# isgasho/h2o-kubernetes

Measured on AMD Instinct MI355X. Metric: GBM train rows/sec on HIGGS-shape 11M×28 at 1/2/4/8 MI355X; AUC parity, higher is better.
Workload: dtype fp32 gradients/hessians; histograms in fixed-point int32 (stochastic rounding) summed exactly in int64; fp64 split gains; exact int64 leaf sums; uint8 bins; 1 GPU; model=GBM bernoulli, global_batch=11000000, rows_per_gpu=11000000, cols=28, max_depth=5, nbins=255, parallelism=dp1

## Files before the change

### h2omx/csrc/tree_kernels.hip

```cpp
#include "common.h"
#include "p2p_device.h"
#include <math.h>

#include <algorithm>
#include <cstdlib>

namespace {

struct SplitParams {
  int mode;
  int leaf_mode;
  int F;
  int is_last_level;
  double min_rows;
  double min_child_weight;
  double lambda_;
  double alpha;
  double gamma;
  double min_split_improvement;
  double learn_rate;
  double max_abs_leaf;
  uint32_t seed;
  int tree_index;
  int depth;
// ... 635 lines not shown
    }
    const unsigned long long bal = __ballot(do_split);
    if (i < n)
      lf_write_node(i, s, do_split, __popcll(bal & ((1ull << lane) - 1ull)), base, next_base, p, nbt, lv, writer,
                    ps_s + i);
    if (lane == 0) {
      int ks = __popcll(bal);
      if (writer) lf_write_ctl(lv.ctl_next, ks, next_base, lv.max_next_nodes);
      if (2 * ks > lv.max_next_nodes) ks = lv.max_next_nodes / 2;
      *res_s = ks;
    }
  }
  __syncthreads();
  return *res_s;
}

struct LevelFin {
  LevelOut lv;
  int* ticket;
};

template <int MODE>
__device__ void level_fin_records(const FeatBest* __restrict__ fbest, const int* __restrict__ ctl, const SplitParams& p,
                                  int nbt, const LevelOut& lv) {
  const int n = ctl[CTL_N];
  const int lane = threadIdx.x & 63, wid = threadIdx.x >> 6, nw = blockDim.x >> 6;
  for (int node = wid; node < n; node += nw) node_best_wave<MODE>(fbest, p.F, node, lane, lv.nsplit);
  __syncthreads();
  level_finalize_body(ctl, p, nbt, lv);
}

constexpr int CMP_STAGE_BYTES = 2048;
constexpr int HB_PF = 1;

template <int NBT, int ROWS, int PKM, bool ROUTE, bool CMP, int COP = 1, bool NID16 = false>
__global__ __launch_bounds__(1024) void hist_build_kernel(
    const uint8_t* __restrict__ codes, int64_t npad, const float* __restrict__ g, const float* __restrict__ s2,
    const int* __restrict__ nid, const NodeLink* __restrict__ link, const int* __restrict__ ctl,
    const int* __restrict__ nvb, const double* __restrict__ qscale, uint32_t salt, int F, int fg, int n_groups,
    int wgpg, int slot_lo, int slot_cnt, const short* __restrict__ slot16, unsigned long long* __restrict__ pk_buf,
    unsigned long long* __restrict__ partials, const PartInfo* __restrict__ part_prev,
    const int* __restrict__ ctl_prev, int* __restrict__ nid_out, int writer, GradFuse gf, LevelPro lp,
    const uint8_t* __restrict__ joint, const int* __restrict__ plane_src) {
  salt = (uint32_t)qscale[9];
  extern __shared__ __attribute__((aligned(16))) unsigned long long lds64[];
  __shared__ int width_s[256], rep_s[256];
  __shared__ float rcp_s[256];
  __shared__ NodeSplit pro_ns[ROUTE ? PRO_MAX_NODES : 1];
  __shared__ PartInfo pro_ps[ROUTE ? PRO_MAX_NODES : 1];
  __shared__ int pro_res;
  bool pro = false;
  if constexpr (ROUTE) pro = lp.fbest != nullptr;
  int n_slots;
  if (pro) n_slots = level_prologue(lp, ctl_prev, NBT, blockIdx.x == 0 && writer != 0, pro_ns, pro_ps, &pro_res);
  else n_slots = ctl[CTL_SLOTS];
  const int b = blockIdx.x;
  const int xcd = b & 7, i = b >> 3;
  const int group = i % n_groups;
  const int chunk = xcd + 8 * (i / n_groups);
  const bool route_w = ROUTE && writer && group == 0 && ctl_prev[CTL_N] > 0;
  const bool build = slot_lo < n_slots;
  if (!build && !route_w) return;
  const int f0 = group * fg;
  const int nf = min(fg, F - f0);
  static_assert(COP == 1 || ((PKM == 1 || PKM == 3 || PKM == 6) && !ROUTE && !CMP), "copies: level-0 kernel only");
  const int hist_elems = slot_cnt * fg * NBT;
  const int lane = threadIdx.x & 63;
  auto plane_codes = [&](int fi) -> const uint8_t* {
    const int sp = plane_src ? plane_src[f0 + fi] : f0 + fi;
    return sp >= 0 ? codes + (int64_t)sp * npad : joint + (int64_t)(~sp) * npad;
  };

  for (int j = threadIdx.x; j < hist_elems * COP; j += blockDim.x) lds64[j] = 0ull;
  if (threadIdx.x < fg) {
    const int fi = threadIdx.x;
    const int w = (fi < nf) ? nvb[f0 + fi] + 1 : NBT;
    width_s[fi] = w;
    int r = NBT / w;
    r = r < 1 ? 1 : (r > 64 ? 64 : r);
    if (COP > 1) r = 1;
    rep_s[fi] = r;
    rcp_s[fi] = 1.0f / (float)r;
  }
  __shared__ float tval_s[PKM == 5 ? GF_LDS_NODES : 1];
  if constexpr (PKM == 5) {
    if (gf.apply && gf.cap <= GF_LDS_NODES)
      for (int j = threadIdx.x; j < gf.cap; j += blockDim.x) tval_s[j] = gf.tree[j].value;
  }
  const float sg = (float)qscale[0], ss = (float)qscale[1];
  const int64_t rb = (int64_t)qscale[7];
  const int64_t n_rows = (int64_t)qscale[8];
  __syncthreads();

  const int64_t units = npad / ROWS;
  const int64_t u0 = units * chunk / wgpg, u1 = units * (chunk + 1) / wgpg;
  const int64_t ustart = CMP ? u0 + (threadIdx.x & ~63) : u0 + threadIdx.x;
  for (int64_t uu = ustart; uu < u1; uu += blockDim.x) {
    const bool inb = !CMP || uu + lane < u1;
    const int64_t u = CMP ? (inb ? uu + lane : u1 - 1) : uu;
    const int64_t r0 = u * ROWS;
    int s[ROWS];
    bool any = false;
    if constexpr (ROUTE) {
      int nn[ROWS], nx[ROWS];
      if (nid == nullptr) {
#pragma unroll
        for (int k = 0; k < ROWS; ++k) nn[k] = (r0 + k < n_rows) ? 0 : INT32_MIN;
      } else if constexpr (NID16) {
        const short* n16 = reinterpret_cast<const short*>(nid);
#pragma unroll
        for (int q = 0; q < ROWS / 8; ++q) {
          const uint4 v = *reinterpret_cast<const uint4*>(n16 + r0 + 8 * q);
          const uint32_t w4[4] = {v.x, v.y, v.z, v.w};
#pragma unroll
          for (int k = 0; k < 8; ++k) nn[8 * q + k] = (int)(short)(w4[k >> 1] >> (16 * (k & 1)));
        }
      } else {
#pragma unroll
        for (int q = 0; q < ROWS / 4; ++q) {
          const int4 n4 = *reinterpret_cast<const int4*>(nid + r0 + 4 * q);
          nn[4 * q] = n4.x; nn[4 * q + 1] = n4.y; nn[4 * q + 2] = n4.z; nn[4 * q + 3] = n4.w;
        }
      }
#pragma unroll
      for (int k = 0; k < ROWS; ++k) { nx[k] = nn[k]; s[k] = -1; }
      const int n_prev = pro ? min(ctl_prev[CTL_N], PRO_MAX_NODES) : ctl_prev[CTL_N];
// ... 67 lines not shown
          any |= (sl >= 0);
        }
      }
    } else if (nid == nullptr) {
#pragma unroll
      for (int k = 0; k < ROWS; ++k) {
        int sl = (r0 + k < n_rows) ? 0 - slot_lo : -1;
        if (sl >= slot_cnt) sl = -1;
        s[k] = sl;
        any |= (sl >= 0);
      }
    } else {
#pragma unroll
      for (int q = 0; q < ROWS / 4; ++q) {
        const int4 n4 = *reinterpret_cast<const int4*>(nid + r0 + 4 * q);
        const int nn[4] = {n4.x, n4.y, n4.z, n4.w};
#pragma unroll
        for (int k = 0; k < 4; ++k) {
          int sl = -1;
          if (nn[k] >= 0) {
            sl = link[nn[k]].slot - slot_lo;
            if (sl >= slot_cnt) sl = -1;
          }
          s[4 * q + k] = sl;
          any |= (sl >= 0);
        }
      }
    }
    if constexpr (CMP) {
      if (__ballot(any && inb) == 0ull) continue;
    } else {
      if (!any) continue;
    }
    uint32_t pf[HB_PF][ROWS / 4];
    auto load_codes = [&](int fi, uint32_t* cw) {
      const uint8_t* cp = plane_codes(fi) + r0;
      if constexpr (ROWS == 16) {
        const uint4 c4 = *reinterpret_cast<const uint4*>(cp);
        cw[0] = c4.x; cw[1] = c4.y; cw[2] = c4.z; cw[3] = c4.w;
      } else {
        const uint2 c2 = *reinterpret_cast<const uint2*>(cp);
        cw[0] = c2.x; cw[1] = c2.y;
      }
    };
    if constexpr (!CMP) {
#pragma unroll
      for (int q = 0; q < HB_PF; ++q)
        if (q < nf) load_codes(q, pf[q]);
    }
    unsigned long long pk[ROWS];
    if constexpr (PKM == 2) {
#pragma unroll
      for (int q = 0; q < ROWS / 2; ++q) {
        const ulonglong2 p2 = *reinterpret_cast<const ulonglong2*>(pk_buf + r0 + 2 * q);
        pk[2 * q] = p2.x;
        pk[2 * q + 1] = p2.y;
      }
    } else if constexpr (PKM == 4 || PKM == 6) {
      const uint32_t* pk32 = reinterpret_cast<const uint32_t*>(pk_buf);
#pragma unroll
      for (int q = 0; q < ROWS / 4; ++q) {
        const uint4 p4 = *reinterpret_cast<const uint4*>(pk32 + r0 + 4 * q);
        const uint32_t pw[4] = {p4.x, p4.y, p4.z, p4.w};
#pragma unroll
        for (int k = 0; k < 4; ++k)
          pk[4 * q + k] = ((unsigned long long)(uint32_t)(int)(short)(pw[k] >> 16) << 32) |
                          (unsigned long long)(pw[k] & 0xFFFFu);
      }
    } else if constexpr (PKM == 5) {
#pragma unroll
      for (int q = 0; q < ROWS / 4; ++q) {
        const float4 f4 = *reinterpret_cast<const float4*>(gf.F + r0 + 4 * q);
        const float4 y4 = *reinterpret_cast<const float4*>(gf.y + r0 + 4 * q);
        int4 n4 = make_int4(-1, -1, -1, -1);
        if (gf.apply) n4 = *reinterpret_cast<const int4*>(gf.nid + r0 + 4 * q);
        float fv[4] = {f4.x, f4.y, f4.z, f4.w};
        const float yv[4] = {y4.x, y4.y, y4.z, y4.w};
        const int nv[4] = {n4.x, n4.y, n4.z, n4.w};
        float gv[4], hv[4];
        uint32_t pw[4];
#pragma unroll
        for (int k = 0; k < 4; ++k) {
          const int64_t r = r0 + 4 * q + k;
          gv[k] = 0.f; hv[k] = 0.f; pw[k] = 0u;
          pk[4 * q + k] = 0ull;
          if (r >= n_rows) continue;
          if (gf.apply) fv[k] += (gf.cap <= GF_LDS_NODES) ? tval_s[~nv[k]] : gf.tree[~nv[k]].value;
          dist_grad(gf.gp.dist, fv[k], yv[k], gf.gp, gv[k], hv[k]);
          const uint32_t hsh = row_hash(rb + r, salt);
          const float d1 = (hsh & 0xFFFF) * (1.0f / 65536.0f), d2 = (hsh >> 16) * (1.0f / 65536.0f);
          const int gq = (int)floorf(fmaf(gv[k], sg, d1));
          const uint32_t sq = (uint32_t)floorf(fmaf(gf.s_is_h ? hv[k] : 1.0f, ss, d2));
          pk[4 * q + k] = ((unsigned long long)(uint32_t)gq << 32) | (unsigned long long)sq;
          pw[k] = ((uint32_t)gq << 16) | (sq & 0xFFFFu);
        }
        if (group == 0) {
          if (gf.apply) *reinterpret_cast<float4*>(gf.F + r0 + 4 * q) = make_float4(fv[0], fv[1], fv[2], fv[3]);
          *reinterpret_cast<float4*>(gf.g + r0 + 4 * q) = make_float4(gv[0], gv[1], gv[2], gv[3]);
          *reinterpret_cast<float4*>(gf.h + r0 + 4 * q) = make_float4(hv[0], hv[1], hv[2], hv[3]);
          if (gf.pk64) {
            *reinterpret_cast<ulonglong2*>(pk_buf + r0 + 4 * q) = make_ulonglong2(pk[4 * q], pk[4 * q + 1]);
            *reinterpret_cast<ulonglong2*>(pk_buf + r0 + 4 * q + 2) = make_ulonglong2(pk[4 * q + 2], pk[4 * q + 3]);
          } else {
            *reinterpret_cast<uint4*>(reinterpret_cast<uint32_t*>(pk_buf) + r0 + 4 * q) =
                make_uint4(pw[0], pw[1], pw[2], pw[3]);
          }
        }
      }
    } else {
#pragma unroll
    for (int q = 0; q < ROWS / 4; ++q) {
      const float4 g4 = *reinterpret_cast<const float4*>(g + r0 + 4 * q);
      float4 s4 = make_float4(1.f, 1.f, 1.f, 1.f);
      if (s2) s4 = *reinterpret_cast<const float4*>(s2 + r0 + 4 * q);
      const float gv[4] = {g4.x, g4.y, g4.z, g4.w};
      const float sv[4] = {s4.x, s4.y, s4.z, s4.w};
#pragma unroll
      for (int k = 0; k < 4; ++k) {
        const uint32_t hsh = row_hash(rb + r0 + 4 * q + k, salt);
        const float d1 = (hsh & 0xFFFF) * (1.0f / 65536.0f), d2 = (hsh >> 16) * (1.0f / 65536.0f);
        const int gq = (int)floorf(fmaf(gv[k], sg, d1));
        const uint32_t sq = (uint32_t)floorf(fmaf(sv[k], ss, d2));
        pk[4 * q + k] = ((unsigned long long)(uint32_t)gq << 32) | (unsigned long long)sq;
      }
    }
    if (PKM == 1 && group == 0) {
#pragma unroll
      for (int q = 0; q < ROWS / 2; ++q)
        *reinterpret_cast<ulonglong2*>(pk_buf + r0 + 2 * q) = make_ulonglong2(pk[2 * q], pk[2 * q + 1]);
    }
    if (PKM == 3 && group == 0) {
      uint32_t* pk32 = reinterpret_cast<uint32_t*>(pk_buf);
#pragma unroll
      for (int q = 0; q < ROWS / 4; ++q) {
        uint32_t pw[4];
#pragma unroll
        for (int k = 0; k < 4; ++k) {
          const unsigned long long v = pk[4 * q + k];
          pw[k] = ((uint32_t)(v >> 32) << 16) | ((uint32_t)v & 0xFFFFu);
        }
        *reinterpret_cast<uint4*>(pk32 + r0 + 4 * q) = make_uint4(pw[0], pw[1], pw[2], pw[3]);
      }
    }
    }
    if constexpr (CMP) {
      static_assert(ROWS == 16 && (PKM == 2 || PKM == 4), "compaction: 16-row units reading stored rows");
      uint32_t m = 0;
#pragma unroll
      for (int r = 0; r < ROWS; ++r)
        if (inb && s[r] >= 0 && pk[r] != 0ull) m |= 1u << r;
      const uint32_t cnt = __popc(m);
      const unsigned long long lt = (1ull << lane) - 1ull;
      int excl = 0, total = 0;
#pragma unroll
      for (int bit = 0; bit < 5; ++bit) {
        const unsigned long long bm = __ballot((cnt >> bit) & 1u);
        excl += __popcll(bm & lt) << bit;
// ... 1644 lines not shown
  if (level_out == nullptr) return false;
  lv = *reinterpret_cast<const LevelOut*>(level_out);
  return lv.ctl_next != nullptr && lv.nvb != nullptr && lv.part != nullptr && lv.tree != nullptr &&
         lv.nsplit != nullptr;
}

static bool make_pro(LevelPro& lp, const void* fbest, const void* params, const void* level_out, int max_nodes) {
  if (fbest == nullptr || params == nullptr || max_nodes < 1 || max_nodes > PRO_MAX_NODES) return false;
  lp.fbest = reinterpret_cast<const FeatBest*>(fbest);
  lp.p = *reinterpret_cast<const SplitParams*>(params);
  return copy_level_out(lp.lv, level_out);
}

static int hist_build_launch(const uint8_t* codes, int64_t npad, const float* g, const float* s2, const int* nid,
                             const void* link, const int* ctl, const int* nvb, const double* qscale, int salt,
                             int F, int nbt, int fg, int n_groups, int wgpg, int slot_lo, int slot_cnt,
                             int rows_per_lane, int threads, const short* slot16, unsigned long long* pk_buf,
                             int pkm, unsigned long long* partials, const void* part_prev, const int* ctl_prev,
                             int* nid_out, int writer, hipStream_t stream, const GradFuse* gfp = nullptr,
                             const LevelPro* lpp = nullptr, const uint8_t* joint = nullptr,
                             const int* plane_src = nullptr) {
  if ((joint == nullptr) != (plane_src == nullptr)) return kBadArg;
  const bool route = part_prev != nullptr;
  GradFuse gfz{};
  if (gfp) gfz = *gfp;
  LevelPro lpz{};
  if (lpp) lpz = *lpp;
  if (lpp && (!route || !writer || lpz.fbest == nullptr || lpz.lv.nsplit == nullptr || lpz.lv.ctl_next != ctl ||
              (const void*)lpz.lv.part != part_prev))
    return kBadArg;
  const bool cmp = (pkm & 8) != 0;
  const int cop = (pkm & 16) ? 8 : ((pkm & 32) ? 4 : 1);
  const bool nid16 = (pkm & 64) != 0;
  pkm &= 7;
  if (nid16 && (!route || cmp || rows_per_lane != 16)) return kBadArg;
  if (cop > 1 && ((pkm != 1 && pkm != 3 && pkm != 6) || route || cmp)) return kBadArg;
  if (pkm == 6 && (nid != nullptr || route || cmp || pk_buf == nullptr)) return kBadArg;
  if (cmp && ((pkm != 2 && pkm != 4) || rows_per_lane != 16 || slot_cnt > 64)) return kBadArg;
  if (route && (ctl_prev == nullptr || nid_out == nullptr || nid_out == nid || (pkm != 2 && pkm != 4)))
    return kBadArg;
  const PartInfo* pp = reinterpret_cast<const PartInfo*>(part_prev);
  if (wgpg % 8 != 0 || npad % 16 != 0 || fg > 256 || threads % 64 != 0 || threads > 1024 || threads < fg)
    return kBadArg;
  if (pkm < 0 || pkm > 6 || (pkm > 0 && pk_buf == nullptr) || ((pkm == 2 || pkm == 4) && !route && slot16 == nullptr))
    return kBadArg;
  if ((pkm == 5) != (gfp != nullptr) || (pkm == 5 && (nid != nullptr || route || cmp || gfz.F == nullptr ||
                                                      gfz.y == nullptr || gfz.g == nullptr || gfz.h == nullptr ||
                                                      (gfz.apply && (gfz.nid == nullptr || gfz.tree == nullptr)))))
    return kBadArg;
  const int64_t units = npad / rows_per_lane;
  if ((units + wgpg - 1) / wgpg * rows_per_lane > ROWS_CAP) return kBadArg;
  const size_t lds = (size_t)slot_cnt * fg * nbt * cop * sizeof(unsigned long long) +
                     (cmp ? (size_t)(threads / 64) * CMP_STAGE_BYTES : 0);
  if (lds > 156 * 1024) return kBadArg;
  const int grid = n_groups * wgpg;
  const NodeLink* lk = reinterpret_cast<const NodeLink*>(link);
#define LAUNCH_HBK(NB, R, M, RT, C)                                                                           \
  hipLaunchKernelGGL((hist_build_kernel<NB, R, M, RT, C>), dim3(grid), dim3(threads), lds, stream, codes, npad, \
                     g, s2, nid, lk, ctl, nvb, qscale, (uint32_t)salt, F, fg, n_groups, wgpg, slot_lo, slot_cnt,  \
                     slot16, pk_buf, partials, pp, ctl_prev, nid_out, writer, gfz, lpz, joint, plane_src)
#define LAUNCH_HBKC(NB, R, M, CP)                                                                                \
  hipLaunchKernelGGL((hist_build_kernel<NB, R, M, false, false, CP>), dim3(grid), dim3(threads), lds, stream, codes, \
                     npad, g, s2, nid, lk, ctl, nvb, qscale, (uint32_t)salt, F, fg, n_groups, wgpg, slot_lo,        \
                     slot_cnt, slot16, pk_buf, partials, pp, ctl_prev, nid_out, writer, gfz, lpz, joint, plane_src)
#define LAUNCH_HBK16(NB, M)                                                                                      \
  hipLaunchKernelGGL((hist_build_kernel<NB, 16, M, true, false, 1, true>), dim3(grid), dim3(threads), lds, stream, \
                     codes, npad, g, s2, nid, lk, ctl, nvb, qscale, (uint32_t)salt, F, fg, n_groups, wgpg, slot_lo,    \
                     slot_cnt, slot16, pk_buf, partials, pp, ctl_prev, nid_out, writer, gfz, lpz, joint, plane_src)
#define LAUNCH_HB(NB, R)                                            \
  do {                                                             \
    if (pkm == 0) LAUNCH_HBK(NB, R, 0, false, false);               \
    else if (pkm == 1 && cop == 8) LAUNCH_HBKC(NB, R, 1, 8);        \
    else if (pkm == 3 && cop == 8) LAUNCH_HBKC(NB, R, 3, 8);        \
    else if (pkm == 1 && cop == 4) LAUNCH_HBKC(NB, R, 1, 4);        \
    else if (pkm == 3 && cop == 4) LAUNCH_HBKC(NB, R, 3, 4);        \
    else if (pkm == 6 && cop == 8) LAUNCH_HBKC(NB, R, 6, 8);        \
    else if (pkm == 6 && cop == 4) LAUNCH_HBKC(NB, R, 6, 4);        \
    else if (pkm == 6) LAUNCH_HBK(NB, R, 6, false, false);          \
    else if (pkm == 1) LAUNCH_HBK(NB, R, 1, false, false);          \
    else if (pkm == 2 && route) LAUNCH_HBK(NB, R, 2, true, false);  \
    else if (pkm == 2) LAUNCH_HBK(NB, R, 2, false, false);          \
    else if (pkm == 3) LAUNCH_HBK(NB, R, 3, false, false);          \
    else if (pkm == 5) LAUNCH_HBK(NB, R, 5, false, false);          \
    else if (route) LAUNCH_HBK(NB, R, 4, true, false);              \
    else LAUNCH_HBK(NB, R, 4, false, false);                        \
  } while (0)
#define LAUNCH_HBCMP(NB)                                             \
  do {                                                              \
    if (pkm == 2 && route) LAUNCH_HBK(NB, 16, 2, true, true);        \
    else if (pkm == 2) LAUNCH_HBK(NB, 16, 2, false, true);           \
    else if (route) LAUNCH_HBK(NB, 16, 4, true, true);               \
    else LAUNCH_HBK(NB, 16, 4, false, true);                         \
  } while (0)
  if (cmp) {
    switch (nbt) {
      case 32: LAUNCH_HBCMP(32); break;
      case 64: LAUNCH_HBCMP(64); break;
      case 128: LAUNCH_HBCMP(128); break;
      case 256: LAUNCH_HBCMP(256); break;
      default: return kBadArg;
    }
  } else if (nid16) {
    switch (nbt) {
      case 32: if (pkm == 2) LAUNCH_HBK16(32, 2); else LAUNCH_HBK16(32, 4); break;
      case 64: if (pkm == 2) LAUNCH_HBK16(64, 2); else LAUNCH_HBK16(64, 4); break;
      case 128: if (pkm == 2) LAUNCH_HBK16(128, 2); else LAUNCH_HBK16(128, 4); break;
      case 256: if (pkm == 2) LAUNCH_HBK16(256, 2); else LAUNCH_HBK16(256, 4); break;
      default: return kBadArg;
    }
  } else if (rows_per_lane == 16) {
    switch (nbt) {
      case 32: LAUNCH_HB(32, 16); break;
      case 64: LAUNCH_HB(64, 16); break;
      case 128: LAUNCH_HB(128, 16); break;
      case 256: LAUNCH_HB(256, 16); break;
      default: return kBadArg;
    }
  } else if (rows_per_lane == 8) {
    switch (nbt) {
      case 32: LAUNCH_HB(32, 8); break;
      case 64: LAUNCH_HB(64, 8); break;
      case 128: LAUNCH_HB(128, 8); break;
      case 256: LAUNCH_HB(256, 8); break;
      default: return kBadArg;
    }
  } else {
    return kBadArg;
  }
#undef LAUNCH_HB
#undef LAUNCH_HBK16
#undef LAUNCH_HBCMP
#undef LAUNCH_HBK
#undef LAUNCH_HBKC
  return launch_status();
}

H2OMX_API int h2omx_hist_build(const uint8_t* codes, int64_t npad, const float* g, const float* s2, const int* nid,
                               const void* link, const int* ctl, const int* nvb, const double* qscale, int salt,
                               int F, int nbt, int fg, int n_groups, int wgpg, int slot_lo, int slot_cnt,
                               int rows_per_lane, int threads, const short* slot16, unsigned long long* pk_buf,
                               int pkm, unsigned long long* partials, const uint8_t* joint,
                               const int* plane_src, hipStream_t stream) {
  return hist_build_launch(codes, npad, g, s2, nid, link, ctl, nvb, qscale, salt, F, nbt, fg, n_groups, wgpg, slot_lo,
                           slot_cnt, rows_per_lane, threads, slot16, pk_buf, pkm, partials, nullptr, nullptr, nullptr,
                           0, stream, nullptr, nullptr, joint, plane_src);
}

H2OMX_API int h2omx_hist_build_grad(const uint8_t* codes, int64_t npad, const int* ctl, const int* nvb,
                                    const double* qscale, int salt, int F, int nbt, int fg, int n_groups, int wgpg,
                                    int slot_cnt, int rows_per_lane, int threads, unsigned long long* pk_buf,
                                    unsigned long long* partials, float* Fm, const float* y, const int* nid_leaf,
                                    const void* tree, int cap, float* g, float* h, int apply, int s_is_h,
                                    int pk64, const void* gparams, const uint8_t* joint, const int* plane_src,
                                    hipStream_t stream) {
  if (gparams == nullptr) return kBadArg;
  GradFuse gf{};
  gf.F = Fm; gf.y = y; gf.nid = nid_leaf; gf.tree = reinterpret_cast<const TreeNode*>(tree);
  gf.g = g; gf.h = h; gf.apply = apply; gf.s_is_h = s_is_h; gf.pk64 = pk64; gf.cap = cap;
  gf.gp = *reinterpret_cast<const GradParams*>(gparams);
  return hist_build_launch(codes, npad, nullptr, nullptr, nullptr, nullptr, ctl, nvb, qscale, salt, F, nbt, fg,
                           n_groups, wgpg, 0, slot_cnt, rows_per_lane, threads, nullptr, pk_buf, 5, partials, nullptr,
                           nullptr, nullptr, 0, stream, &gf, nullptr, joint, plane_src);
// ... 2535 lines not shown
```

### h2omx/models/tree/engine.py

```python
from __future__ import annotations

import ctypes
import math
import os
from dataclasses import dataclass, field

import numpy as np
import torch

from ... import ops
from .binning import BinnedMatrix
from ...utils.trace import PhaseTimer
from .structs import (FEAT_BEST_BYTES, NODE_LINK_BYTES, NODE_SPLIT_BYTES, PART_INFO_BYTES, TREE_NODE_DTYPE, GradParams,
                      LevelOut, SplitParams, check_layout, interaction_masks)


@dataclass
class TreeParams:
    max_depth: int = 5
    min_rows: float = 10.0
    min_child_weight: float = 0.0
    reg_lambda: float = 0.0
    reg_alpha: float = 0.0
    gamma: float = 0.0
# ... 17 lines not shown

def tree_capacity(max_depth: int) -> int:
    return (1 << (max_depth + 1)) - 1


class HipTreeBuilder:

    LDS_BUDGET = 64 * 1024
    THREADS = 1024
    TARGET_WGS = 512
    ROWS_PER_LANE = 16
    ROWS_CAP = 262144
    SYNC_NODE_CAP = 4096
    SEG_TARGET_CHUNKS = 1024
    SEG_LDS_BUDGET = 16 * 1024
    SEG_LDS_BUDGET_WIDE = 64 * 1024
    SCAN_SLOTS = 1
    MEAN_LEAVES_NO_H = True
    BAG_COMPACT = True
    bag_compact = False
    DEEP_DEPTH = 10
    FUSE_MAX_DEPTH = 8
    FUSE_MAX_PREV = 4
    CLOSE_SINGLE_BLOCK = 2048
    DIRECT_MIN_NODES = 2048
    DIRECT_MAX_ELIG = 32.0
    DIRECT_WAVE_ROWS = 512
    PART_WAVE_NODES = 2048
    DIRECT_CHUNKED = True
    PART_BLOCKS = 1024
    FUSE_ROUTE = True
    BUNDLE = True
    PK32 = True
    FUSE_GRAD = False
    CHAIN_BEGIN = True
    LEAF_REPS = 16
    FUSE_FIN = True
    FUSE_FIN_LOCAL = False
    FIN_PROLOGUE = True
    FIN_PROLOGUE_FINAL = False
    PERMUTE_GS = True
    ECODES = True
    LF_MULTI_BLOCK = True
    COLMAJOR_EVERY = 0

    def __init__(self, bm: BinnedMatrix, params: TreeParams, comm=None):
        if not bm.codes.is_cuda:
            raise ValueError("HipTreeBuilder needs device-resident codes")
        self.lib = ops.tree_lib()
        check_layout(self.lib)
        self.bm = bm
        self.p = params
        self.comm = comm
        self.dev = bm.codes.device
        self.F = bm.F
        self.nbt = bm.nbt
        self.per_node = self.F * 2 * self.nbt
        if params.max_depth < 1:
            raise ValueError("max_depth must be >= 1")
        self.capacity = tree_capacity(min(params.max_depth, 24))
        d = self.dev
        self.ctl = torch.zeros((2, 4), dtype=torch.int32, device=d)
        self.ctl_init = torch.tensor([1, 1, 0, 1], dtype=torch.int32, device=d)
        self.link_init = torch.tensor([0, -1, -1, 0], dtype=torch.int32, device=d)
        self._bufs: dict[str, torch.Tensor] = {}
        self.tree_buf = torch.zeros((self.capacity * TREE_NODE_DTYPE.itemsize,), dtype=torch.uint8, device=d)
# ... 74 lines not shown
        self.planes = None
        if self.BUNDLE and not self.segmented and (comm is None or comm.world_size <= 1):
            self.planes = bm.bundle
        self.n_planes = self.planes.P if self.planes is not None else self.F

    def _hist_planes(self):
        pl = self.planes
        if pl is None:
            return self.F, self.bm.nvb, None, None, None
        return pl.P, pl.plane_nvb_dev, pl.joint, pl.plane_src_dev, pl.feat_plane_dev

    def _ticket_buf(self, numel: int) -> torch.Tensor:
        t = getattr(self, "_tickets", None)
        if t is None or t.numel() < numel:
            t = self._tickets = torch.zeros(max(numel, 1024), dtype=torch.int32, device=self.dev)
        return t

    def _lf_tiles(self, max_nodes: int) -> int:
        if not self.LF_MULTI_BLOCK:
            return 0
        return self._buf("lf_tiles", max_nodes // 1024 + 2, torch.int32).data_ptr()

    def _buf(self, name: str, numel: int, dtype) -> torch.Tensor:
        b = self._bufs.get(name)
        if b is None or b.numel() < numel:
            b = torch.empty((max(numel, 1),), dtype=dtype, device=self.dev)
            self._bufs[name] = b
        return b

    DEEP_LDS_BUDGET = 128 * 1024
    DEEP_MIN_GROUPS = 4
    L0_COPIES = 8

    def plan_l0(self):
        key = ("l0", self.L0_COPIES)
        if key not in self.plans:
            self.plans[key] = self._plan(1, self.DEEP_LDS_BUDGET, self.THREADS, mult=self.L0_COPIES)
        return self.plans[key]

    N_CUS = 256
    MIN_GROUPS = 1
    P2P_BLOCKS = 256
    MAX_WG_THREADS_PER_CU = 2048

    def _fill_rounds(self, wgpg: int, n_groups: int, lds_bytes: int, threads: int, units: int) -> int:
        per_cu = max(1, min((160 * 1024) // max(1, lds_bytes + 3072), self.MAX_WG_THREADS_PER_CU // threads))
        resident = self.N_CUS * per_cu
        total = n_groups * wgpg
        if total <= resident:
            return wgpg
        rounds = math.ceil(total / resident)
        fill = (rounds * resident // n_groups) // 8 * 8
        if fill > wgpg and fill * threads <= units:
            return fill
        return wgpg

    SMALL_SHARD = True
    FILL_ROUNDS = True

    def _plan(self, max_slots: int, budget: int, threads: int, units: int | None = None, mult: int = 1):
        per_slot_feat = self.nbt * 8 * mult
        F = getattr(self, "n_planes", None) or self.F
        if max_slots * per_slot_feat <= budget:
            slot_cnt = max_slots
            fg_max = max(1, min(F, 256, budget // (max_slots * per_slot_feat)))
            n_groups = math.ceil(F / fg_max)
            fg = math.ceil(F / n_groups)
            passes = 1
        else:
            fg, n_groups = 1, F
            slot_cnt = max(1, budget // per_slot_feat)
            passes = math.ceil(max_slots / slot_cnt)
        if passes == 1 and self.MIN_GROUPS > n_groups and mult == 1:
            fg = math.ceil(F / min(F, self.MIN_GROUPS))
            n_groups = math.ceil(F / fg)
        if units is None:
            units = self.bm.npad // self.ROWS_PER_LANE

        def target(t: int) -> int:
            return max(8, (self.TARGET_WGS * 512 // t // n_groups) // 8 * 8)

        def grid(t: int, upl: int) -> int:
            return min(target(t), max(8, (units // (t * upl)) // 8 * 8))

        wgpg = grid(threads, 2)
        if self.SMALL_SHARD and n_groups * wgpg < self.N_CUS and wgpg < target(threads):
            wgpg = grid(threads, 1)
            if n_groups * wgpg < self.N_CUS and passes == 1:
                ng = min(F, math.ceil(self.N_CUS / wgpg))
                if ng > n_groups:
                    fg = math.ceil(F / ng)
                    n_groups = math.ceil(F / fg)
                    wgpg = grid(threads, 1)
        cap =self.ROWS_CAP if self.max_rows_per_wg is None else min(self.ROWS_CAP, self.max_rows_per_wg)
        min_wgpg = math.ceil(math.ceil(units / (cap // self.ROWS_PER_LANE)) / 8) * 8
        wgpg = max(wgpg, min_wgpg)
        if self.FILL_ROUNDS:
            wgpg = self._fill_rounds(wgpg, n_groups, slot_cnt * fg * per_slot_feat, threads, units)
        return dict(slot_cnt=slot_cnt, fg=fg, n_groups=n_groups, passes=passes, wgpg=wgpg, threads=threads)

    def plan_level(self, max_slots: int):
        key = max_slots
        if key in self.plans:
            return self.plans[key]
        plan = self._choose(max_slots)
        self.plans[key] = plan
        return plan

    def _choose(self, max_slots: int, units: int | None = None):
        lo, hi = self.LDS_BUDGET, self.DEEP_LDS_BUDGET
        plan = self._plan(max_slots, lo, self.THREADS, units)
        if hi > lo and plan["n_groups"] >= self.DEEP_MIN_GROUPS:
            deep = self._plan(max_slots, hi, 1024, units)
            if deep["n_groups"] < plan["n_groups"] or deep["passes"] < plan["passes"]:
                plan = deep
        return plan

    def _fused_level(self, d: int) -> bool:
        return (1 << (d - 1)) <= self.FUSE_MAX_PREV

    def _params(self, tree_index: int):
        p, sp = self.p, self._sp
        sp.mode, sp.leaf_mode, sp.F, sp.is_last_level = p.mode, p.leaf_mode, self.F, 0
        sp.min_rows, sp.min_child_weight = p.min_rows, p.min_child_weight
        sp.lambda_, sp.alpha, sp.gamma = p.reg_lambda, p.reg_alpha, p.gamma
        sp.min_split_improvement, sp.learn_rate, sp.max_abs_leaf = p.min_split_improvement, p.learn_rate, p.max_abs_leaf
        sp.seed, sp.tree_index = p.seed & 0xFFFFFFFF, tree_index
        sp.col_rate, sp.mtries = p.col_sample_rate, p.mtries
        sp.mono = self.mono.data_ptr() if self.mono is not None else None
        sp.gbound = self.gbound.data_ptr() if self.gbound is not None else None
        sp.ifsets = self.ifsets.data_ptr() if self.ifsets is not None else None
        sp.istate = self.istate.data_ptr() if self.istate is not None else None
        sp.catf = self.catf.data_ptr() if self.catf is not None else None
        sp.treecat = self.treecat.data_ptr() if self.treecat is not None else None
        sp.fbcat = None
        sp.hist_mode, sp.hist_top, sp.hist_nbins = p.hist_mode, p.hist_top, p.hist_nbins
        sp.edges = self.bm.edges.data_ptr() if p.hist_mode else None
        sp.frange = self._frange.data_ptr() if p.hist_mode else None
        return ctypes.addressof(sp)

    def _level_out(self, ctl_nxt, part, nl, nsplit, next_nodes: int) -> LevelOut:
        P = ops.P
        return LevelOut(P(ctl_nxt), P(self.bm.edges), P(self.bm.nvb), P(part), P(nl), P(self.tree_buf), P(nsplit),
                        next_nodes, self.capacity)

    def _cat_level(self, max_nodes: int) -> None:
# ... 28 lines not shown
        s2 = w if p.mode == 0 else h
        link = [self._buf("link0", 4, torch.int32), None]
        T = self.timer.phase
        if not chain:
            with T("tree_begin"):
                self.begin(smax, tree_index)
        pk_boost = chain and self.pk_in_boost
        full_prev = None
        max_depth = p.max_depth
        final_ctl = self.ctl[max_depth % 2]
        max_nodes = 1
        fuse = self.fuse_route
        nid16 = self.nid16 is not None
        nid_buf = self.nid16 if nid16 else (self.nid, self.nid2)
        part_prev = None
        pend = None
        for d in range(max_depth):
            cur, nxt = d % 2, (d + 1) % 2
            ctl_cur, ctl_nxt = self.ctl[cur], self.ctl[nxt]
            if max_nodes > self.SYNC_NODE_CAP:
                n_now, s_now = [int(v) for v in ctl_cur[:2].tolist()]
                self.stats["host_syncs"] += 1
                if n_now == 0:
                    final_ctl = ctl_cur
                    break
                max_nodes, max_slots = n_now, s_now
            else:
                max_slots = 1 if d == 0 else max(1, max_nodes // 2)
            last = d == max_depth - 1
            plan = self.plan_level(max_slots)
            l0_copies = d == 0 and grad_fuse is None and self.L0_COPIES in (4, 8)
            if l0_copies:
                plan = self.plan_l0()
            built = self._buf("built", max_slots * self.per_node, torch.int64)
            full_cur = None if last else self._buf(f"full{cur}", max_nodes * self.per_node, torch.int64)
            sp.depth = d
            sp.children_leaves = 1 if last else 0
            self._cat_level(max_nodes)
            fuse_p2p = (p2p is not None
                        and max_slots * nbt * 8 <= self.LDS_BUDGET
                        and max_slots * -(-F // p2p.world) * p2p.world * 2 * nbt * 8 <= p2p.cap
                        and 2 * max_slots * F * FEAT_BEST_BYTES <= p2p.cap // 2)
            rs = comm is None or fuse_p2p
            fbest = self._buf("fbest", max_nodes * F * FEAT_BEST_BYTES // 8, torch.float64)
            next_nodes = 2 * max_nodes
            part = self._buf("part", max_nodes * PART_INFO_BYTES // 4, torch.int32)
            nl = None
            if not last:
                nl = self._buf(f"link{nxt}", next_nodes * NODE_LINK_BYTES // 4, torch.int32)
                link[nxt] = nl
            nsplit = self._buf("nsplit", max_nodes * NODE_SPLIT_BYTES // 8, torch.float64)
            fin = rs and max_nodes <= 64 and ((fuse_p2p and self.FUSE_FIN)
                                              or (comm is None and self.FUSE_FIN_LOCAL and plan["passes"] == 1))
            if fin and getattr(self, "_fin_ticket", None) is None:
                self._fin_ticket = torch.zeros((1,), dtype=torch.int32, device=self.dev)
            lvo = self._level_out(ctl_nxt, part, nl, nsplit, next_nodes)
            pro = None
            if (self.FIN_PROLOGUE and comm is None and fuse and not fin and plan["passes"] == 1
                    and max_nodes <= 64):
                if last:
                    pro = "final" if self.FIN_PROLOGUE_FINAL else None
                elif not self._fused_level(d + 1):
                    pro = "route"
                elif self.plan_level(max(1, next_nodes // 2))["passes"] == 1:
                    pro = "hist"

# ... 40 lines not shown
                            P(joint), P(plane_src), st),
                            "hist_build_route_fin")
                        pend = None
                    elif d > 0 and fuse and self._fused_level(d):
                        ops.check(lib.h2omx_hist_build_route(
                            P(bm.codes), bm.npad, P(None if (d == 1 and self.implicit_root) else nid_buf[(d - 1) % 2]),
                            P(part_prev), P(ctl_nxt),
                            P(nid_buf[d % 2]), 1 if ps == 0 else 0, P(ctl_cur), P(nvb_h), P(self.qscale), Fh, nbt,
                            plan["fg"], plan["n_groups"], plan["wgpg"], slot_lo, plan["slot_cnt"],
                            self.ROWS_PER_LANE, plan["threads"], P(self.pk),
                            (4 if self.pk32 else 2) + (64 if nid16 else 0),
                            P(partials), P(joint), P(plane_src), st),
                            "hist_build_route")
                    elif d == 0 and grad_fuse is not None:
                        gf = grad_fuse
                        ops.check(lib.h2omx_hist_build_grad(
                            P(bm.codes), bm.npad, P(ctl_cur), P(nvb_h), P(self.qscale), tree_index & 0x7FFFFFFF,
                            Fh, nbt, plan["fg"], plan["n_groups"], plan["wgpg"], plan["slot_cnt"],
                            self.ROWS_PER_LANE, plan["threads"], P(self.pk), P(partials), P(gf["F"]), P(gf["y"]),
                            P(self.nid), P(self.tree_buf), self.capacity, P(g), P(h), 1 if gf["apply"] else 0,
                            0 if p.mode == 0 else 1, 0 if self.pk32 else 1, ctypes.addressof(gf["gp"]),
                            P(joint), P(plane_src), st),
                            "hist_build_grad")
                    else:
                        ops.check(lib.h2omx_hist_build(
                            P(bm.codes), bm.npad, P(g), P(s2),
                            P(None if (d == 0 and self.implicit_root) else (nid_buf[d % 2] if fuse else self.nid)),
                            P(link[cur]), P(ctl_cur), P(nvb_h),
                            P(self.qscale), tree_index & 0x7FFFFFFF, Fh, nbt, plan["fg"], plan["n_groups"],
                            plan["wgpg"], slot_lo, plan["slot_cnt"], self.ROWS_PER_LANE, plan["threads"],
                            P(self.slot16), P(self.pk),
                            ((6 if pk_boost else 1 + (2 if self.pk32 else 0)) if d == 0
                             else 2 + (2 if self.pk32 else 0))
                            + ({8: 16, 4: 32}.get(self.L0_COPIES, 0) if l0_copies else 0),
                            P(partials), P(joint), P(plane_src), st),
                            "hist_build")
                with T("hist_reduce"):
                    reduce(plan["n_groups"], plan["wgpg"], plan["fg"], slot_lo, plan["slot_cnt"])
            if comm is not None and not fuse_p2p:
                with T("allreduce"):
                    comm.all_reduce_(built[: max_slots * self.per_node])
            with T("split"):
                if not rs:
                    ops.check(lib.h2omx_split_find(P(built), P(full_prev), P(full_cur), P(ctl_cur),
                                                   P(link[cur]), P(bm.nvb), P(tree_fmask), P(self.qscale), spp,
                                                   max_nodes, nbt, P(fbest), st), "split_find")
                if fin:
                    pass
                elif pro is not None:
                    spc = type(sp).from_buffer_copy(sp)
                    pro_args = (P(fbest), ctypes.addressof(spc), ctypes.addressof(lvo), max_nodes)
                    if pro == "hist":
                        pend = dict(args=pro_args, keep=(spc, lvo, fbest, nl, nsplit, self._bufs.get("fbcat")))
                elif fuse_p2p:
                    ops.check(lib.h2omx_node_best_finalize_p2p(p2p.desc_ptr, P(ctl_cur), spp, nbt,
                                                               ctypes.addressof(lvo), st), "node_best_finalize_p2p")
                else:
                    ops.check(lib.h2omx_level_finalize(P(fbest), P(ctl_cur), spp, nbt, ctypes.addressof(lvo),
                                                       max_nodes, self._lf_tiles(max_nodes), st), "level_finalize")
            win = min(3 * max_nodes, self.capacity)
            with T("partition"):
                if fuse and last:
                    rg = self.regrad if (chain and w is None) else None
                    leaf16 = chain and nid16
                    self.leaf16_buf = nid_buf[(d + 1) % 2] if leaf16 else None
                    pf_args = (P(bm.codes), bm.npad, P(nid_buf[d % 2]),
                               P(self.leaf16_buf if leaf16 else self.nid),
# ... 439 lines not shown
```

Measured before the change: 16.19 billion rows/s (row-trees per second, all GPUs).

## Batch all feature-group code loads per row unit in level-0 histogram build

```diff
diff --git a/h2omx/csrc/tree_kernels.hip b/h2omx/csrc/tree_kernels.hip
--- a/h2omx/csrc/tree_kernels.hip
+++ b/h2omx/csrc/tree_kernels.hip
@@ -691,8 +691,22 @@
 
 constexpr int CMP_STAGE_BYTES = 2048;
 constexpr int HB_PF = 1;
-
-template <int NBT, int ROWS, int PKM, bool ROUTE, bool CMP, int COP = 1, bool NID16 = false>
+constexpr int FG_MAX = 8;
+
+__device__ __forceinline__ unsigned long long pk_widen(uint32_t pw) {
+  return ((unsigned long long)(uint32_t)(int)(short)(pw >> 16) << 32) | (unsigned long long)(pw & 0xFFFFu);
+}
+
+__device__ __forceinline__ unsigned long long pk_quantise(float gv, float sv, float sg, float ss, int64_t row,
+                                                          uint32_t salt) {
+  const uint32_t hsh = row_hash(row, salt);
+  const float d1 = (hsh & 0xFFFF) * (1.0f / 65536.0f), d2 = (hsh >> 16) * (1.0f / 65536.0f);
+  const int gq = (int)floorf(fmaf(gv, sg, d1));
+  const uint32_t sq = (uint32_t)floorf(fmaf(sv, ss, d2));
+  return ((unsigned long long)(uint32_t)gq << 32) | (unsigned long long)sq;
+}
+
+template <int NBT, int ROWS, int PKM, bool ROUTE, bool CMP, int COP = 1, bool NID16 = false, bool BATCH = false>
 __global__ __launch_bounds__(1024) void hist_build_kernel(
     const uint8_t* __restrict__ codes, int64_t npad, const float* __restrict__ g, const float* __restrict__ s2,
     const int* __restrict__ nid, const NodeLink* __restrict__ link, const int* __restrict__ ctl,
@@ -751,6 +765,23 @@
   const int64_t n_rows = (int64_t)qscale[8];
   __syncthreads();
 
+  static_assert(!BATCH || (!ROUTE && !CMP && (PKM == 1 || PKM == 3 || PKM == 6) && ROWS == 16),
+                "batched loop: level 0 (one slot: the launcher checks)");
+  constexpr int NQ = BATCH ? FG_MAX : 1;
+  const uint8_t* pbase[NQ];
+  int rep_q[NQ], width_q[NQ];
+  float rcp_q[NQ];
+  if constexpr (BATCH) {
+#pragma unroll
+    for (int q = 0; q < NQ; ++q) {
+      const int fi = min(q, nf - 1);
+      pbase[q] = plane_codes(fi);
+      rep_q[q] = __builtin_amdgcn_readfirstlane(rep_s[fi]);
+      width_q[q] = __builtin_amdgcn_readfirstlane(width_s[fi]);
+      rcp_q[q] = __int_as_float(__builtin_amdgcn_readfirstlane(__float_as_int(rcp_s[fi])));
+    }
+  }
+
   const int64_t units = npad / ROWS;
   const int64_t u0 = units * chunk / wgpg, u1 = units * (chunk + 1) / wgpg;
   const int64_t ustart = CMP ? u0 + (threadIdx.x & ~63) : u0 + threadIdx.x;
@@ -884,6 +915,93 @@
     } else {
       if (!any) continue;
     }
+    if constexpr (BATCH) {
+      uint32_t live = 0;
+#pragma unroll
+      for (int r = 0; r < ROWS; ++r) live |= (s[r] >= 0 ? 1u : 0u) << r;
+      unsigned long long pk[ROWS];
+      uint4 raw4[PKM == 6 ? ROWS / 4 : 1];
+      float4 rawg[PKM == 6 ? 1 : ROWS / 4], raws[PKM == 6 ? 1 : ROWS / 4];
+      if constexpr (PKM == 6) {
+#pragma unroll
+        for (int q = 0; q < ROWS / 4; ++q)
+          raw4[q] = *reinterpret_cast<const uint4*>(reinterpret_cast<const uint32_t*>(pk_buf) + r0 + 4 * q);
+      } else {
+#pragma unroll
+        for (int q = 0; q < ROWS / 4; ++q) {
+          rawg[q] = *reinterpret_cast<const float4*>(g + r0 + 4 * q);
+          raws[q] = make_float4(1.f, 1.f, 1.f, 1.f);
+          if (s2) raws[q] = *reinterpret_cast<const float4*>(s2 + r0 + 4 * q);
+        }
+      }
+      uint4 cq[NQ];
+#pragma unroll
+      for (int q = 0; q < NQ; ++q) cq[q] = *reinterpret_cast<const uint4*>(pbase[q] + r0);
+      __builtin_amdgcn_sched_barrier(0);
+      if constexpr (PKM == 6) {
+#pragma unroll
+        for (int q = 0; q < ROWS / 4; ++q) {
+          const uint32_t pw[4] = {raw4[q].x, raw4[q].y, raw4[q].z, raw4[q].w};
+#pragma unroll
+          for (int k = 0; k < 4; ++k) pk[4 * q + k] = pk_widen(pw[k]);
+        }
+      } else {
+#pragma unroll
+        for (int q = 0; q < ROWS / 4; ++q) {
+          const float gv[4] = {rawg[q].x, rawg[q].y, rawg[q].z, rawg[q].w};
+          const float sv[4] = {raws[q].x, raws[q].y, raws[q].z, raws[q].w};
+#pragma unroll
+          for (int k = 0; k < 4; ++k) pk[4 * q + k] = pk_quantise(gv[k], sv[k], sg, ss, rb + r0 + 4 * q + k, salt);
+        }
+        if (group == 0) {
+          if constexpr (PKM == 1) {
+#pragma unroll
+            for (int q = 0; q < ROWS / 2; ++q)
+              *reinterpret_cast<ulonglong2*>(pk_buf + r0 + 2 * q) = make_ulonglong2(pk[2 * q], pk[2 * q + 1]);
+          } else {
+            uint32_t* pk32 = reinterpret_cast<uint32_t*>(pk_buf);
+#pragma unroll
+            for (int q = 0; q < ROWS / 4; ++q) {
+              uint32_t pw[4];
+#pragma unroll
+              for (int k = 0; k < 4; ++k) {
+                const unsigned long long v = pk[4 * q + k];
+                pw[k] = ((uint32_t)(v >> 32) << 16) | ((uint32_t)v & 0xFFFFu);
+              }
+              *reinterpret_cast<uint4*>(pk32 + r0 + 4 * q) = make_uint4(pw[0], pw[1], pw[2], pw[3]);
+            }
+          }
+        }
+      }
+#pragma unroll
+      for (int r = 0; r < ROWS; ++r) pk[r] &= (unsigned long long)(long long)((int)(live << (31 - r)) >> 31);
+#pragma unroll
+      for (int q = 0; q < NQ; ++q) {
+        if (q == 0 || q < nf) {
+          const uint32_t cw[4] = {cq[q].x, cq[q].y, cq[q].z, cq[q].w};
+          if (COP == 1 && rep_q[q] > 1) {
+            const int width = width_q[q];
+            const int copy = lane - rep_q[q] * (int)(((float)lane + 0.5f) * rcp_q[q]);
+            unsigned long long* hb = lds64 + q * NBT + copy * width;
+#pragma unroll
+            for (int r = 0; r < ROWS; ++r) {
+              if (pk[r] != 0ull) {
+                int bin = (cw[r >> 2] >> (8 * (r & 3))) & 0xff;
+                if (bin == NBT - 1) bin = width - 1;
+                atomicAdd(hb + bin, pk[r]);
+              }
+            }
+          } else {
+            unsigned long long* hb = lds64 + q * NBT * COP + (lane & (COP - 1));
+#pragma unroll
+            for (int r = 0; r < ROWS; ++r) atomicAdd(hb + ((cw[r >> 2] >> (8 * (r & 3))) & (NBT - 1)) * COP, pk[r]);
+          }
+        }
+      }
+#pragma unroll
+      for (int q = 1; q < NQ; ++q) __asm__ volatile("" ::"v"(cq[q].x), "v"(cq[q].y), "v"(cq[q].z), "v"(cq[q].w));
+      continue;
+    }
     uint32_t pf[HB_PF][ROWS / 4];
     auto load_codes = [&](int fi, uint32_t* cw) {
       const uint8_t* cp = plane_codes(fi) + r0;
@@ -915,9 +1033,7 @@
         const uint4 p4 = *reinterpret_cast<const uint4*>(pk32 + r0 + 4 * q);
         const uint32_t pw[4] = {p4.x, p4.y, p4.z, p4.w};
 #pragma unroll
-        for (int k = 0; k < 4; ++k)
-          pk[4 * q + k] = ((unsigned long long)(uint32_t)(int)(short)(pw[k] >> 16) << 32) |
-                          (unsigned long long)(pw[k] & 0xFFFFu);
+        for (int k = 0; k < 4; ++k) pk[4 * q + k] = pk_widen(pw[k]);
       }
     } else if constexpr (PKM == 5) {
 #pragma unroll
@@ -968,13 +1084,7 @@
       const float gv[4] = {g4.x, g4.y, g4.z, g4.w};
       const float sv[4] = {s4.x, s4.y, s4.z, s4.w};
 #pragma unroll
-      for (int k = 0; k < 4; ++k) {
-        const uint32_t hsh = row_hash(rb + r0 + 4 * q + k, salt);
-        const float d1 = (hsh & 0xFFFF) * (1.0f / 65536.0f), d2 = (hsh >> 16) * (1.0f / 65536.0f);
-        const int gq = (int)floorf(fmaf(gv[k], sg, d1));
-        const uint32_t sq = (uint32_t)floorf(fmaf(sv[k], ss, d2));
-        pk[4 * q + k] = ((unsigned long long)(uint32_t)gq << 32) | (unsigned long long)sq;
-      }
+      for (int k = 0; k < 4; ++k) pk[4 * q + k] = pk_quantise(gv[k], sv[k], sg, ss, rb + r0 + 4 * q + k, salt);
     }
     if (PKM == 1 && group == 0) {
 #pragma unroll
@@ -2685,7 +2795,10 @@
   const bool cmp = (pkm & 8) != 0;
   const int cop = (pkm & 16) ? 8 : ((pkm & 32) ? 4 : 1);
   const bool nid16 = (pkm & 64) != 0;
+  bool batch = (pkm & 128) != 0;
   pkm &= 7;
+  if (route || cmp || (pkm != 1 && pkm != 3 && pkm != 6) || fg > FG_MAX || rows_per_lane != 16 || slot_cnt != 1)
+    batch = false;
   if (nid16 && (!route || cmp || rows_per_lane != 16)) return kBadArg;
   if (cop > 1 && ((pkm != 1 && pkm != 3 && pkm != 6) || route || cmp)) return kBadArg;
   if (pkm == 6 && (nid != nullptr || route || cmp || pk_buf == nullptr)) return kBadArg;
@@ -2720,6 +2833,23 @@
   hipLaunchKernelGGL((hist_build_kernel<NB, 16, M, true, false, 1, true>), dim3(grid), dim3(threads), lds, stream, \
                      codes, npad, g, s2, nid, lk, ctl, nvb, qscale, (uint32_t)salt, F, fg, n_groups, wgpg, slot_lo,    \
                      slot_cnt, slot16, pk_buf, partials, pp, ctl_prev, nid_out, writer, gfz, lpz, joint, plane_src)
+#define LAUNCH_HBB(NB, M, CP)                                                                                    \
+  hipLaunchKernelGGL((hist_build_kernel<NB, 16, M, false, false, CP, false, true>), dim3(grid), dim3(threads), lds, \
+                     stream, codes, npad, g, s2, nid, lk, ctl, nvb, qscale, (uint32_t)salt, F, fg, n_groups, wgpg,    \
+                     slot_lo, slot_cnt, slot16, pk_buf, partials, pp, ctl_prev, nid_out, writer, gfz, lpz, joint,     \
+                     plane_src)
+#define LAUNCH_HBATCH(NB)                                      \
+  do {                                                        \
+    if (pkm == 1 && cop == 8) LAUNCH_HBB(NB, 1, 8);            \
+    else if (pkm == 1 && cop == 4) LAUNCH_HBB(NB, 1, 4);       \
+    else if (pkm == 1) LAUNCH_HBB(NB, 1, 1);                   \
+    else if (pkm == 3 && cop == 8) LAUNCH_HBB(NB, 3, 8);       \
+    else if (pkm == 3 && cop == 4) LAUNCH_HBB(NB, 3, 4);       \
+    else if (pkm == 3) LAUNCH_HBB(NB, 3, 1);                   \
+    else if (cop == 8) LAUNCH_HBB(NB, 6, 8);                   \
+    else if (cop == 4) LAUNCH_HBB(NB, 6, 4);                   \
+    else LAUNCH_HBB(NB, 6, 1);                                 \
+  } while (0)
 #define LAUNCH_HB(NB, R)                                            \
   do {                                                             \
     if (pkm == 0) LAUNCH_HBK(NB, R, 0, false, false);               \
@@ -2745,7 +2875,15 @@
     else if (route) LAUNCH_HBK(NB, 16, 4, true, true);               \
     else LAUNCH_HBK(NB, 16, 4, false, true);                         \
   } while (0)
-  if (cmp) {
+  if (batch) {
+    switch (nbt) {
+      case 32: LAUNCH_HBATCH(32); break;
+      case 64: LAUNCH_HBATCH(64); break;
+      case 128: LAUNCH_HBATCH(128); break;
+      case 256: LAUNCH_HBATCH(256); break;
+      default: return kBadArg;
+    }
+  } else if (cmp) {
     switch (nbt) {
       case 32: LAUNCH_HBCMP(32); break;
       case 64: LAUNCH_HBCMP(64); break;
@@ -2781,6 +2919,8 @@
     return kBadArg;
   }
 #undef LAUNCH_HB
+#undef LAUNCH_HBATCH
+#undef LAUNCH_HBB
 #undef LAUNCH_HBK16
 #undef LAUNCH_HBCMP
 #undef LAUNCH_HBK
diff --git a/h2omx/models/tree/engine.py b/h2omx/models/tree/engine.py
--- a/h2omx/models/tree/engine.py
+++ b/h2omx/models/tree/engine.py
@@ -73,6 +73,8 @@
     FUSE_ROUTE = True
     BUNDLE = True
     PK32 = True
+    HIST_BATCH = True
+    HIST_FG_MAX = 8
     FUSE_GRAD = False
     CHAIN_BEGIN = True
     LEAF_REPS = 16
@@ -213,10 +215,10 @@
     DEEP_MIN_GROUPS = 4
     L0_COPIES = 8
 
-    def plan_l0(self):
-        key = ("l0", self.L0_COPIES)
+    def plan_l0(self, fg_cap: int | None = None):
+        key = ("l0", self.L0_COPIES, fg_cap)
         if key not in self.plans:
-            self.plans[key] = self._plan(1, self.DEEP_LDS_BUDGET, self.THREADS, mult=self.L0_COPIES)
+            self.plans[key] = self._plan(1, self.DEEP_LDS_BUDGET, self.THREADS, mult=self.L0_COPIES, fg_cap=fg_cap)
         return self.plans[key]
 
     N_CUS = 256
@@ -239,7 +241,8 @@
     SMALL_SHARD = True
     FILL_ROUNDS = True
 
-    def _plan(self, max_slots: int, budget: int, threads: int, units: int | None = None, mult: int = 1):
+    def _plan(self, max_slots: int, budget: int, threads: int, units: int | None = None, mult: int = 1,
+              fg_cap: int | None = None):
         per_slot_feat = self.nbt * 8 * mult
         F = getattr(self, "n_planes", None) or self.F
         if max_slots * per_slot_feat <= budget:
@@ -255,6 +258,9 @@
         if passes == 1 and self.MIN_GROUPS > n_groups and mult == 1:
             fg = math.ceil(F / min(F, self.MIN_GROUPS))
             n_groups = math.ceil(F / fg)
+        if fg_cap is not None and fg > fg_cap:
+            n_groups = math.ceil(F / fg_cap)
+            fg = math.ceil(F / n_groups)
         if units is None:
             units = self.bm.npad // self.ROWS_PER_LANE
 
@@ -280,19 +286,19 @@
             wgpg = self._fill_rounds(wgpg, n_groups, slot_cnt * fg * per_slot_feat, threads, units)
         return dict(slot_cnt=slot_cnt, fg=fg, n_groups=n_groups, passes=passes, wgpg=wgpg, threads=threads)
 
-    def plan_level(self, max_slots: int):
-        key = max_slots
+    def plan_level(self, max_slots: int, fg_cap: int | None = None):
+        key = max_slots if fg_cap is None else (max_slots, fg_cap)
         if key in self.plans:
             return self.plans[key]
-        plan = self._choose(max_slots)
+        plan = self._choose(max_slots, fg_cap=fg_cap)
         self.plans[key] = plan
         return plan
 
-    def _choose(self, max_slots: int, units: int | None = None):
+    def _choose(self, max_slots: int, units: int | None = None, fg_cap: int | None = None):
         lo, hi = self.LDS_BUDGET, self.DEEP_LDS_BUDGET
-        plan = self._plan(max_slots, lo, self.THREADS, units)
+        plan = self._plan(max_slots, lo, self.THREADS, units, fg_cap=fg_cap)
         if hi > lo and plan["n_groups"] >= self.DEEP_MIN_GROUPS:
-            deep = self._plan(max_slots, hi, 1024, units)
+            deep = self._plan(max_slots, hi, 1024, units, fg_cap=fg_cap)
             if deep["n_groups"] < plan["n_groups"] or deep["passes"] < plan["passes"]:
                 plan = deep
         return plan
@@ -387,6 +393,11 @@
             l0_copies = d == 0 and grad_fuse is None and self.L0_COPIES in (4, 8)
             if l0_copies:
                 plan = self.plan_l0()
+            batch = (self.HIST_BATCH and d == 0 and grad_fuse is None and self.ROWS_PER_LANE == 16
+                     and plan["passes"] == 1)
+            if batch and plan["fg"] > self.HIST_FG_MAX:
+                plan = (self.plan_l0(self.HIST_FG_MAX) if l0_copies
+                        else self.plan_level(max_slots, self.HIST_FG_MAX))
             built = self._buf("built", max_slots * self.per_node, torch.int64)
             full_cur = None if last else self._buf(f"full{cur}", max_nodes * self.per_node, torch.int64)
             sp.depth = d
@@ -493,7 +504,8 @@
                             P(self.slot16), P(self.pk),
                             ((6 if pk_boost else 1 + (2 if self.pk32 else 0)) if d == 0
                              else 2 + (2 if self.pk32 else 0))
-                            + ({8: 16, 4: 32}.get(self.L0_COPIES, 0) if l0_copies else 0),
+                            + ({8: 16, 4: 32}.get(self.L0_COPIES, 0) if l0_copies else 0)
+                            + (128 if batch else 0),
                             P(partials), P(joint), P(plane_src), st),
                             "hist_build")
                 with T("hist_reduce"):
```

New measurement: 16.51 billion rows/s (row-trees per second, all GPUs), median of 6. +2.0%, better.
